# 9to1url/PairPhone

Measured on AMD Instinct MI355X. Metric: MELPe-1200 channel-seconds encoded/sec (node), higher is better.
Workload: dtype int16/int32 saturating fixed point; 1 GPU; config 4: 262144 channels per GPU, melpe_a per superframe (NPP x3 + MELPe-1200 analysis + 81-bit packing); channels_per_gpu=262144, channels_total=262144, parallelism=channel shards, 1 GPU(s), no collective

## Files before the change

pairphone_amd/build.py:

```python
import os
import subprocess
import sys

ROOT = os.path.dirname(os.path.dirname(os.path.abspath(__file__)))
CSRC = os.path.join(ROOT, "pairphone_amd", "csrc")
LIB = os.path.join(ROOT, "pairphone_amd", "libmelpe_amd.so")
EMU = os.path.join(ROOT, "build", "libmelpe_hostemu.so")
REF = "/root/reference/melpe"
HIPCC = os.environ.get("HIPCC", "/opt/rocm/bin/hipcc")
ARCH = os.environ.get("MELPE_ARCH", "gfx950")


def _run(cmd, **kw):
    print("+", " ".join(cmd), flush=True)
    subprocess.run(cmd, check=True, **kw)


def _newer(target, deps):
    if not os.path.exists(target):
        return True
    t = os.path.getmtime(target)
    return any(os.path.getmtime(d) > t for d in deps if os.path.exists(d))


def _sources():
    out = []
    for d in (CSRC, os.path.join(ROOT, "include")):
        for f in os.listdir(d):
            if f.endswith((".h", ".hip", ".cpp")):
                out.append(os.path.join(d, f))
    out.append(os.path.join(ROOT, "pairphone_amd", "data", "melpe_tables.bin"))
    return out


def build_oracle():
    if not os.path.isdir(REF):
        print("reference not present: using prebuilt oracle/_ref and committed tables")
        return
    _run(["make", "-s", "-C", os.path.join(ROOT, "oracle"), "-j8"])
    _run([sys.executable, os.path.join(ROOT, "oracle", "dump_tables.py")])


PROF_LIB = os.path.join(ROOT, "pairphone_amd", "libmelpe_amd_prof.so")


TUS = ("engine", "k_npp", "k_ana", "k_ana_mw", "k_harm", "k_dec", "k_r24", "k_dsp_eval", "k_par",
       "k_link")
HOT_TUS = ("k_npp", "k_ana", "k_ana_mw", "k_harm", "k_dec", "k_r24", "k_dsp_eval", "k_par", "k_link")
TU_FLAGS = {"k_ana": ["-mllvm", "-amdgpu-disable-unclustered-high-rp-reschedule"]}


def build_engine(force=False, prof=False, defs=(), out=None, tus_defs=None, hot=HOT_TUS, only=None):
    out = out or (PROF_LIB if prof else LIB)
    deps = _sources()
    if not force and not _newer(out, deps):
        return out
    blob = os.path.join(ROOT, "pairphone_amd", "data", "melpe_tables.bin")
    tag = os.path.splitext(os.path.basename(out))[0]
    objdir = os.path.join(ROOT, "build", "obj", tag)
    os.makedirs(objdir, exist_ok=True)
    common = [HIPCC, "-O3", "--offload-arch=" + ARCH, "-std=c++17", "-fPIC", "-c",
              "-Wno-unused-result", "-Wno-unused-value", '-DMELPE_TABLES_BIN="%s"' % blob] \
        + (["-DMELPE_PROF"] if prof else []) + ["-D" + d for d in defs] \
        + os.environ.get("MELPE_EXTRA_FLAGS", "").split()
    procs, objs = [], []
    for tu in TUS:
        o = os.path.join(objdir, tu + ".o")
        objs.append(o)
        if only is not None and tu not in only and os.path.exists(o):
            continue
        extra = (["-DMELPE_INLINE_ALL"] if tu in hot else []) + TU_FLAGS.get(tu, [])
        if tus_defs and tu in tus_defs:
            extra += ["-D" + d for d in tus_defs[tu]]
        cmd = common + extra + [os.path.join(CSRC, tu + ".hip"), "-o", o]
        print("+", " ".join(cmd), flush=True)
        procs.append((tu, subprocess.Popen(cmd)))
    bad = [tu for tu, p in procs if p.wait() != 0]
    if bad:
        raise RuntimeError("hipcc failed for " + ", ".join(bad))
    check_no_flat(objdir)
    tmp = out + ".tmp"
# ... 1 lines not shown
    os.replace(tmp, out)
    return out


LLVM_BIN = "/opt/rocm/lib/llvm/bin"


def device_disassembly(obj, arch=None):
    arch = arch or ARCH
    import tempfile
    with tempfile.TemporaryDirectory() as tmp:
        fat, elf = os.path.join(tmp, "fat.bin"), os.path.join(tmp, "dev.elf")
        subprocess.run(["objcopy", "--dump-section", ".hip_fatbin=" + fat, obj], check=True)
        for a in dict.fromkeys((arch, "gfx950")):
            r = subprocess.run([os.path.join(LLVM_BIN, "clang-offload-bundler"), "--unbundle", "--type=o",
                                "--input=" + fat, "--targets=hipv4-amdgcn-amd-amdhsa--" + a,
                                "--output=" + elf], capture_output=True)
            if r.returncode == 0 and os.path.getsize(elf) > 0:
                break
        else:
            raise RuntimeError("no gfx950 code object in " + obj)
        txt = subprocess.run([os.path.join(LLVM_BIN, "llvm-objdump"), "-d", "--no-show-raw-insn",
                              elf], check=True, capture_output=True, text=True).stdout
    out, cur = {}, None
    for line in txt.splitlines():
        if line.endswith(">:") and "<" in line:
            cur = line[line.index("<") + 1:-2]
            out[cur] = []
        elif cur and line.startswith("\t"):
            out[cur].append(line.strip())
    return out


NO_FLAT = ("k_enc_ana", "k_enc_harm", "k_enc_tail", "k_decode", "k_vad", "k_enc_npp", "k_npp",
           "k_demodulate", "k_enc24",
           "k_dec24", "k_helpers_eval", "k_stream", "k_dsp_eval", "k_parse", "k_par_tap")


def check_no_flat(objdir):
    bad = []
    for f in sorted(os.listdir(objdir)):
        if not f.endswith(".o"):
            continue
        for sym, ins in device_disassembly(os.path.join(objdir, f)).items():
            if any(k in sym for k in NO_FLAT):
                n = sum(1 for i in ins if i.startswith("flat_"))
                if n:
                    bad.append("%s: %d flat_ instructions" % (sym, n))
    if bad:
        raise RuntimeError("generic FLAT accesses in codec kernels: " + "; ".join(bad))


def build_hostemu(force=False):
    deps = _sources()
    if not force and not _newer(EMU, deps):
        return EMU
    os.makedirs(os.path.dirname(EMU), exist_ok=True)
    tmp = EMU + ".tmp"
    _run(["g++", "-O2", "-std=c++17", "-shared", "-fPIC", "-I" + CSRC,
          os.path.join(CSRC, "hostemu.cpp"), "-o", tmp])
    os.replace(tmp, EMU)
    return EMU


def build_opcount(force=False):
    out = os.path.join(ROOT, "build", "libmelpe_opcount.so")
    if not force and not _newer(out, _sources()):
# ... 32 lines not shown
```

pairphone_amd/csrc/encoder.h:

```cpp
#ifndef MELPE_ENCODER_H
#define MELPE_ENCODER_H

#include "quant.h"

namespace mlp {



MD void ana_first(EncAna *E)
{
	if (!E->ana_started) {
		v_zero(E->lpfsp_delin, LPF_ORD);
		v_zero(E->lpfsp_delout, LPF_ORD);
		E->pitch_avg = DEFAULT_PITCH_Q7;
		v_set(E->fpitch, DEFAULT_PITCH_Q7, 2);
		E->ana_started = 1;
	}
}

MN Word16 global_pitch(const int16_t *speech, int16_t *sb, int16_t *delin, int16_t *delout)
{
	Word16 dontcare;
#if !defined(MELPE_OPCOUNT)
	{
// ... 417 lines not shown
	window(E->sigbuf, TB(win_cof), E->sigbuf, LPC_FRAME);
	find_harm_fft(E->sigbuf, hb, LPC_FRAME);
}

MN void ana_pack(EncAna *E)
{
	MelpParam *par = E->par;
	quant_fsmag(E, par);
	for (int i = 0; i < NF; i++)
		E->qpar.uv_flag[i] = par[i].uv_flag;
	low_rate_chn_write(E);
	v_copy(E->hpspeech, &E->hpspeech[NF * FRAME], IN_BEG);
}

MN void analysis_tail(EncAna *E)
{
	MelpParam *par = E->par;
	sc_ana(E, par);
#if !defined(MELPE_KO_LSFVQ)
	lsf_vq(E, par);
#endif
	pitch_vq(E, par);
	gain_vq(E, par);
	for (int i = 0; i < NF; i++)
		quant_u(&par[i].jitter, &E->qpar.jit_index[i], 0, MAX_JITTER_Q15, 2, SW_MAX_,
			true, 7);
	quant_bp(E, par);
	quant_jitter(E, par);
	for (int i = 0; i < NF; i++)
		ana_fsmag_frame(E, &par[i], i);
	ana_pack(E);
}

MN void analysis_a2(EncAna *E, int16_t *res)
{
	MelpParam *par = E->par;
	sc_ana(E, par);
#if !defined(MELPE_KO_LSFVQ)
	lsf_vq(E, par);
#endif
	ANA_CKPT(4);
	pitch_vq(E, par);
	gain_vq(E, par);
	for (int i = 0; i < NF; i++)
		quant_u(&par[i].jitter, &E->qpar.jit_index[i], 0, MAX_JITTER_Q15, 2, SW_MAX_,
			true, 7);
	quant_bp(E, par);
	quant_jitter(E, par);
	for (int i = 0; i < NF; i++) {
		if (par[i].uv_flag)
			continue;
		int16_t lpc[LPC_ORD + 1];
		lpc[0] = 4096;
		lpc_lsp2pred(par[i].lsf, &lpc[1], LPC_ORD);
		zerflt(&E->hpspeech[i * FRAME + FRAME_END - LPC_FRAME / 2], lpc, E->sigbuf, LPC_ORD,
		       LPC_FRAME);
		window(E->sigbuf, TB(win_cof), E->sigbuf, LPC_FRAME);
		v_copy(&res[i * LPC_FRAME], E->sigbuf, LPC_FRAME);
	}
	v_copy(E->hpspeech, &E->hpspeech[NF * FRAME], IN_BEG);
}

MN void analysis_a(EncAna *E, const int16_t *sp_in, int16_t *res)
{
#if defined(MELPE_KO_ANALYSIS)
	return;
#endif
	for (int i = 0; i < NF; i++) {
		analysis_frame(E, sp_in, i);
		ANA_CKPT(i + 1);
	}
	analysis_a2(E, res);
}

MD void ana_shift(EncAna *E)
{
	v_copy(E->hpspeech, &E->hpspeech[NF * FRAME], IN_BEG);
}

MN void analysis_b(EncAna *E)
{
	MelpParam *par = E->par;
	quant_fsmag(E, par);
	for (int i = 0; i < NF; i++)
		E->qpar.uv_flag[i] = par[i].uv_flag;
	low_rate_chn_write(E);
}

MN void analysis(EncAna *E, const int16_t *sp_in)
{
	PROF_SCOPE(15);
#if defined(MELPE_KO_ANALYSIS)
	return;
#endif
	for (int i = 0; i < NF; i++)
		analysis_frame(E, sp_in, i);
	analysis_tail(E);
}

MN void analysis_upto(EncAna *E, const int16_t *sp_in, int upto)
{
	MelpParam *par = E->par;
	int16_t lpc[LPC_ORD + 1];
	for (int i = 0; i < NF; i++) {
		dc_rmv(&sp_in[i * FRAME], &E->hpspeech[IN_BEG + i * FRAME], E->dcdelin,
// ... 53 lines not shown
```

pairphone_amd/csrc/engine.hip:

```cpp
#include <hip/hip_runtime.h>
#include <stdio.h>
#include <stdlib.h>
#include <string.h>
#include <stdint.h>
#include <initializer_list>
#include <string>
#include <mutex>
#include <vector>

#include "kern.h"
#define SYN_FN __host__ __device__ static inline
#include "synth.h"
#include "voice_crypt.h"
#include "vad.h"
#include "stream_fmt.h"
#include "ops_eval.h"
#include "helpers_eval.h"
#include "dsp_eval_modes.h"
#define MODEM_FN __host__ __device__ static inline
#include "modem.h"
#include "../../include/melpe.h"
#include "../../include/melpe_batch.h"

#if !defined(__HIP_DEVICE_COMPILE__)
// ... 486 lines not shown
	hipEvent_t done = nullptr;
	hipStream_t last = nullptr;
	bool used = false;
};

static hipError_t bin_alloc(BinBuf *b, int channels)
{
	size_t pb = sizeof(int) * (size_t) channels, cb = sizeof(unsigned) * (2 * NBIN + 4);
	const size_t kb = sizeof(uint16_t) * (size_t) channels;
	char *p = nullptr;
	hipError_t er = hipMalloc(&p, pb + cb + kb);
	if (er != hipSuccess)
		return er;
	er = hipEventCreateWithFlags(&b->done, hipEventDisableTiming);
	if (er != hipSuccess) {
		hipFree(p);
		return er;
	}
	b->perm = (int *) p;
	b->ctl = (unsigned *) (p + pb);
	b->key = (uint16_t *) (p + pb + cb);
	return hipMemset(b->ctl, 0, cb);
}

__device__ __forceinline__ int bin_class(const char *rec, int off_par, int off_uv)
{
	const int16_t *uv = (const int16_t *) (rec + off_uv);
	const int nv = (uv[0] == 0) + (uv[1] == 0) + (uv[2] == 0);
	int b = (*(const int16_t *) (rec + off_par + (NF - 1) * sizeof(MelpParam)) >> 7) - 20;
	b = b < 0 ? 0 : (b > BIN_PITCHES - 1 ? BIN_PITCHES - 1 : b);
	return nv * BIN_PITCHES + b;
}

__global__ __launch_bounds__(256) void k_bin_count(const char *rec, size_t stride, int off_par,
						   int off_uv, const uint8_t *active, int n, BinBuf b)
{
	__shared__ unsigned cnt[NBIN];
	for (int k = threadIdx.x; k < NBIN; k += blockDim.x)
		cnt[k] = 0;
	__syncthreads();
	int c = blockIdx.x * blockDim.x + threadIdx.x;
	if (c < n) {
		int k = NOT_LIVE;
		if (!active || active[c]) {
			k = bin_class(rec + (size_t) c * stride, off_par, off_uv);
			atomicAdd(&cnt[k], 1u);
		}
		b.key[c] = (uint16_t) k;
	}
	__syncthreads();
	for (int k = threadIdx.x; k < NBIN; k += blockDim.x)
		if (cnt[k])
			atomicAdd(&b.ctl[k], cnt[k]);
}

__global__ void k_bin_scan(BinBuf b)
{
	if (threadIdx.x == 0) {
		unsigned acc = 0;
		for (int k = 0; k < NBIN; k++) {
			b.ctl[NBIN + k] = acc;
			acc += b.ctl[k];
		}
		b.ctl[2 * NBIN] = acc;
		b.ctl[2 * NBIN + 1] = 0;
		b.ctl[2 * NBIN + 2] = 0;
	}
}

__global__ __launch_bounds__(256) void k_bin_scatter(int n, BinBuf b)
{
	__shared__ unsigned cnt[NBIN], base[NBIN];
	for (int k = threadIdx.x; k < NBIN; k += blockDim.x)
		cnt[k] = 0;
	__syncthreads();
	int c = blockIdx.x * blockDim.x + threadIdx.x;
	int k = c < n ? b.key[c] : NOT_LIVE;
	unsigned r = 0;
	if (k != NOT_LIVE)
		r = atomicAdd(&cnt[k], 1u);
	__syncthreads();
	for (int j = threadIdx.x; j < NBIN; j += blockDim.x)
		if (cnt[j])
			base[j] = atomicAdd(&b.ctl[NBIN + j], cnt[j]);
	__syncthreads();
	if (k != NOT_LIVE)
		b.perm[base[k] + r] = c;
}

static bool bin_enabled(void)
{
	static const bool on = env_int("MELPE_BIN", 1) != 0;
	return on;
}

static hipError_t bin_launch(int order, BinBuf &b, const void *rec, size_t stride, int off_par,
			     int off_uv, const uint8_t *active, int n, hipStream_t s, bool *on)
{
	*on = !(order == 0 || (order < 0 && !bin_enabled()));
	if (!*on)
		return hipSuccess;
	hipError_t er;
	if (b.used && b.last != s && (er = hipStreamWaitEvent(s, b.done, 0)) != hipSuccess)
		return er;
	unsigned g = (unsigned) ((n + 255) / 256);
	if ((er = hipMemsetAsync(b.ctl, 0, sizeof(unsigned) * NBIN, s)) != hipSuccess)
		return er;
	k_bin_count<<<g, 256, 0, s>>>((const char *) rec, stride, off_par, off_uv, active, n, b);
	if ((er = hipGetLastError()) != hipSuccess)
		return er;
	k_bin_scan<<<1, WAVE, 0, s>>>(b);
	if ((er = hipGetLastError()) != hipSuccess)
		return er;
	k_bin_scatter<<<g, 256, 0, s>>>(n, b);
	return hipGetLastError();
}

static hipError_t bin_release(BinBuf &b, hipStream_t s)
{
	b.last = s;
	b.used = true;
	return hipEventRecord(b.done, s);
}

#define MW_MAX_CHANNELS (512 * WAVE)
#define DEC2_MAX_CHANNELS (1024 * WAVE)

struct melpe_engine {
	int device = 0;
	int channels = 0;
	hipStream_t stream = nullptr;
	hipEvent_t ev0 = nullptr, ev1 = nullptr;
	hipEvent_t ev_in = nullptr, ev_out = nullptr;
	hipEvent_t ev_host = nullptr;
	hipEvent_t ev_pin = nullptr, ev_npp = nullptr;
	EncState *d_enc = nullptr;
	DecState *d_dec = nullptr;
	synth_state *d_syn = nullptr;
	int16_t *d_pcm = nullptr;
	unsigned char *d_bits = nullptr;
	uint8_t *d_mask = nullptr;
	int16_t *d_npp = nullptr;
	BinBuf bin_enc, bin_dec;
	int lane_order = -1;
	int ana_waves = 0;
	uint32_t *d_lq = nullptr;
	int dec_waves = 0;
	uint32_t *d_hb = nullptr;
	int mw_live_max = MW_MAX_CHANNELS;
	size_t scratch_need = 0;
	int16_t *d_res = nullptr;
	std::vector<std::pair<hipStream_t, hipEvent_t>> marks;
	std::recursive_mutex mu;
	size_t npp_bytes = 0;
	float last_ms = 0.f;
	struct Slot {
		int16_t *pcm = nullptr;
		unsigned char *bits = nullptr;
		uint8_t *mask = nullptr;
		hipEvent_t loaded = nullptr, done = nullptr, freed = nullptr;
		bool used = false;
	} slot[2];
	hipStream_t cin = nullptr, cout = nullptr;
	hipStream_t cdec = nullptr;
	hipEvent_t ev_dec = nullptr;
	long async_calls = 0;
	hipStream_t own = nullptr;
};

static int ana_waves_for(melpe_engine *e)
{
	if (e->ana_waves == 1 || e->ana_waves == 4)
		return e->ana_waves;
	long groups = (e->channels + WAVE - 1) / WAVE;
	return groups <= 512 ? 4 : 1;
}

static int ana_launch(melpe_engine *e, const int16_t *d_sp, uint8_t *d_bits, const uint8_t *d_act,
		      hipStream_t s, hipEvent_t after_sort = nullptr)
{
	BinBuf &b = e->bin_enc;
	bool on;
	hipError_t er = bin_launch(e->lane_order, b, e->d_enc, sizeof(EncState),
				   (int) (offsetof(EncState, a) + offsetof(EncAna, par)),
				   (int) (offsetof(EncState, a) + offsetof(EncAna, qpar) + offsetof(QuantParam, uv_flag)),
				   d_act, e->channels, s, &on);
	if (er != hipSuccess)
		return (int) er;
	if (after_sort && (er = hipEventRecord(after_sort, s)) != hipSuccess)
		return (int) er;
	const int *perm = on ? b.perm : nullptr;
	const int *nlive = on ? (const int *) (b.ctl + 2 * NBIN) : nullptr;
	int nw = ana_waves_for(e);
	AnaGate all;
	all.tag = (int *) (b.ctl + 2 * NBIN + 1);
	const bool dual = nw == 1 && on && e->ana_waves == 0 && e->mw_live_max > 0;
	AnaGate lane = all, mw = all;
	if (dual) {
		lane.lo = e->mw_live_max;
		mw.hi = e->mw_live_max;
	}
	int rc = 0;
	if (dual || nw == 4)
		rc = kl_enc_ana_mw(e->d_enc, d_sp, d_bits, d_act, e->channels, perm, nlive, e->d_lq, mw, s);
	if (rc == 0 && nw == 1) {
		rc = kl_enc_ana(e->d_enc, d_sp, d_act, e->channels, perm, nlive, e->d_res, lane, s);
		if (rc == 0)
			rc = kl_enc_harm(e->d_enc, e->d_res, d_act, e->channels, perm, nlive, lane, s);
		if (rc == 0)
			rc = kl_enc_tail(e->d_enc, d_bits, d_act, e->channels, perm, nlive, lane, s);
	}
	if (rc == 0 && on)
		rc = (int) bin_release(b, s);
	return rc;
}

static int dec_waves_for(melpe_engine *e)
{
	int nw = e->dec_waves;
	if (nw != 1 && nw != 2)
		nw = e->channels <= DEC2_MAX_CHANNELS ? 2 : 1;
	return nw == 2 && e->d_hb ? 2 : 1;
}

static int dec_launch(melpe_engine *e, int16_t *d_sp, const uint8_t *d_bits, const uint8_t *d_act,
		      hipStream_t s)
{
	BinBuf &b = e->bin_dec;
	bool on;
	hipError_t er = bin_launch(e->lane_order, b, e->d_dec, sizeof(DecState),
				   (int) offsetof(DecState, par),
				   (int) (offsetof(DecState, qpar) + offsetof(QuantParam, uv_flag)),
				   d_act, e->channels, s, &on);
	if (er != hipSuccess)
		return (int) er;
	const int *perm = on ? b.perm : nullptr;
	const int *nlive = on ? (const int *) (b.ctl + 2 * NBIN) : nullptr;
	int rc = dec_waves_for(e) == 2
			 ? kl_decode2(e->d_dec, d_sp, d_bits, d_act, e->channels, perm, nlive, e->d_hb, s)
			 : kl_decode(e->d_dec, d_sp, d_bits, d_act, e->channels, perm, nlive, s);
	if (rc == 0 && on)
		rc = (int) bin_release(b, s);
	return rc;
// ... 270 lines not shown
			HIPCHK(hipStreamWaitEvent(e->cdec, e->ev_pin, 0));
			HIPCHK((hipError_t) dec_launch(e, (int16_t *) dc->sp, (const uint8_t *) dc->bits,
						       (const uint8_t *) dc->active, e->cdec));
			HIPCHK(hipEventRecord(e->ev_dec, e->cdec));
		}
		if (nx) {
			HIPCHK(hipStreamWaitEvent(e->cin, e->ev_pin, 0));
			if (nx->vad)
				if (int r = vad_launch(nx->vad, nx->sp, nx->votes, (void *) nx->mask, nx->active,
						       e->channels, e->cin))
					return r;
			HIPCHK((hipError_t) kl_enc_npp(e->d_enc, (int16_t *) nx->sp, (const uint8_t *) nx->mask,
						       e->channels, e->cin));
			HIPCHK(hipEventRecord(e->ev_npp, e->cin));
			HIPCHK(hipStreamWaitEvent(s, e->ev_npp, 0));
		}
		if (dc)
			HIPCHK(hipStreamWaitEvent(s, e->ev_dec, 0));
		return 0;
	});
}

extern "C" {

const char *melpe_last_error(void)
{
	return g_err.c_str();
}

static int engine_warm(melpe_engine *e)
{
	hipError_t er;
	const int mw = e->channels < MW_MAX_CHANNELS ? e->channels : MW_MAX_CHANNELS;
	int (*warm[])(int, hipStream_t) = {kl_npp_warm, kl_ana_warm, kl_harm_warm, kl_ana_mw_warm, kl_dec_warm};
	for (auto f : warm)
		if ((er = (hipError_t) f(f == kl_ana_mw_warm ? mw : e->channels, e->stream)) != hipSuccess)
			return fail("melpe_engine: codec kernel scratch could not be reserved", er);
	if (e->d_hb && (er = (hipError_t) kl_dec2_warm(e->channels, e->stream)) != hipSuccess)
		return fail("melpe_engine: codec kernel scratch could not be reserved", er);

	if ((er = hipStreamSynchronize(e->stream)) != hipSuccess)
		return fail("melpe_engine: codec kernel scratch could not be reserved", er);
	return 0;
}

static int engine_reserve(melpe_engine *e)
{
	DEVGUARD(e->device);
	hipError_t er;
	if ((er = hipMalloc(&e->d_res, sizeof(int16_t) * NF * LPC_FRAME * (size_t) e->channels)) != hipSuccess) {
		e->d_res = nullptr;
		return fail("melpe_engine_create: analysis residual buffer", er);
	}
	if ((er = hipMalloc(&e->d_lq, sizeof(uint32_t) * kl_enc_ana_mw_lq_words(e->channels))) != hipSuccess) {
		e->d_lq = nullptr;
		return fail("melpe_engine_create: multi-wave score rows", er);
	}
	if (e->channels <= DEC2_MAX_CHANNELS &&
	    (er = hipMalloc(&e->d_hb, sizeof(uint32_t) * kl_decode2_hb_words(e->channels))) != hipSuccess) {
		e->d_hb = nullptr;
		return fail("melpe_engine_create: two-wave decoder hand-over buffers", er);
	}
	const int mw = e->channels < MW_MAX_CHANNELS ? e->channels : MW_MAX_CHANNELS;
	{
		const size_t lane = kl_ana_private() > kl_harm_private() ? kl_ana_private() : kl_harm_private();
		const size_t dec_lane = kl_dec_private() > kl_parse_private() ? kl_dec_private() : kl_parse_private();
		const size_t per_wave = (lane > dec_lane ? lane : dec_lane) * WAVE;
		const size_t mw_wave = kl_ana_mw_private() * WAVE;
		const size_t ww = kl_npp_private() > kl_harm_wave_private() ? kl_npp_private() : kl_harm_wave_private();
		const size_t waves = (size_t) (e->channels + WAVE - 1) / WAVE;
		const size_t mw_waves = 4 * (size_t) ((mw + WAVE - 1) / WAVE);
		size_t resident = (size_t) e->channels;
		hipDeviceProp_t prop;
		if (hipGetDeviceProperties(&prop, e->device) == hipSuccess) {
			const size_t r = (size_t) prop.multiProcessorCount * (size_t) (prop.maxThreadsPerMultiProcessor / WAVE);
			if (r > 0 && r < resident)
				resident = r;
		}
		size_t need = per_wave * waves;
		if (mw_wave * mw_waves > need)
			need = mw_wave * mw_waves;
		if (e->d_hb && kl_dec2_private() * WAVE * 2 * waves > need)
			need = kl_dec2_private() * WAVE * 2 * waves;
		if (ww * WAVE * resident > need)
			need = ww * WAVE * resident;
		size_t cur = 0, mx = 0;
		if (hipDeviceGetLimit(&cur, hipExtLimitScratchCurrent) == hipSuccess &&
		    hipDeviceGetLimit(&mx, hipExtLimitScratchMax) == hipSuccess && need > cur) {
			if (need > mx)
				return fail_msg("melpe_engine_create: the codec kernels' scratch exceeds the "
						"device's scratch limit (fewer channels per engine)");
			if ((er = hipDeviceSetLimit(hipExtLimitScratchCurrent, need)) != hipSuccess)
				return fail("melpe_engine_create: raising the scratch limit", er);
		}
		e->scratch_need = need;
	}
	return engine_warm(e);
}
// ... 2 lines not shown
{
	if (!out || channels <= 0)
		return fail_msg("melpe_engine_create: bad arguments");
	int ndev = 0;
	HIPCHK(hipGetDeviceCount(&ndev));
	if (device < 0 || device >= ndev)
		return fail_msg("melpe_engine_create: no such HIP device");
	int rc = ensure_device_tables(device);
	if (rc)
		return rc;
	DEVGUARD(device);
	melpe_engine *e = new melpe_engine();
	e->device = device;
	e->channels = channels;
	hipError_t er = hipSuccess;
	const char *what = nullptr;
#define CREATE_STEP(expr) if (er == hipSuccess && (er = (expr)) != hipSuccess) what = #expr
	e->stream = g_dev_stream[device];
	CREATE_STEP(hipEventCreate(&e->ev0));
	CREATE_STEP(hipEventCreate(&e->ev1));
	CREATE_STEP(hipEventCreateWithFlags(&e->ev_in, hipEventDisableTiming));
	CREATE_STEP(hipEventCreateWithFlags(&e->ev_out, hipEventDisableTiming));
	CREATE_STEP(hipEventCreateWithFlags(&e->ev_host, hipEventDisableTiming));
	CREATE_STEP(hipEventCreateWithFlags(&e->ev_pin, hipEventDisableTiming));
	CREATE_STEP(hipEventCreateWithFlags(&e->ev_npp, hipEventDisableTiming));
	CREATE_STEP(hipMalloc(&e->d_enc, sizeof(EncState) * (size_t) channels));
	CREATE_STEP(hipMalloc(&e->d_dec, sizeof(DecState) * (size_t) channels));
	CREATE_STEP(hipMalloc(&e->d_syn, sizeof(synth_state) * (size_t) channels));
	CREATE_STEP(hipMalloc(&e->d_pcm, sizeof(int16_t) * MELPE_SF_SAMPLES * (size_t) channels));
	CREATE_STEP(hipMalloc(&e->d_bits, (size_t) MELPE_SF_BYTES * channels));
	CREATE_STEP(hipMalloc(&e->d_mask, (size_t) channels));
	CREATE_STEP(bin_alloc(&e->bin_enc, channels));
	CREATE_STEP(bin_alloc(&e->bin_dec, channels));
#undef CREATE_STEP
	if (er != hipSuccess) {
		int r = fail(what, er);
		melpe_engine_destroy(e);
		return r;
	}
	int r = melpe_engine_reset(e, nullptr, 3);
	if (r == 0)
		r = engine_reserve(e);
	if (r) {
		std::string m = g_err;
		melpe_engine_destroy(e);
		g_err = m;
		return r;
	}
	*out = e;
	return 0;
}

int melpe_engine_set_own_stream(melpe_engine *e, int on)
{
	if (!e)
		return fail_msg("melpe_engine_set_own_stream: null engine");
	DEVGUARD(e->device);
	HOST_LOCK(e);
	ENGINE_WAIT(e);
	HIPCHK(hipStreamSynchronize(e->stream));
	if (on && !e->own) {
		HIPCHK(hipStreamCreateWithFlags(&e->own, hipStreamNonBlocking));
		e->stream = e->own;
		if (int rc = engine_warm(e)) {
			e->stream = g_dev_stream[e->device];
			hipStreamDestroy(e->own);
// ... 43 lines not shown
		return fail_msg("melpe_engine_set_dec_waves: waves must be 0 (auto), 1 or 2");
	if (waves == 2 && !e->d_hb)
		return fail_msg("melpe_engine_set_dec_waves: the two-wave decoder is available up to "
				"65,536 channels per engine");
	std::lock_guard<std::recursive_mutex> lk(e->mu);
	e->dec_waves = waves;
	return 0;
}

int melpe_engine_set_ana_waves(melpe_engine *e, int waves)
{
	if (!e || !(waves == 0 || waves == 1 || waves == 4))
		return fail_msg("melpe_engine_set_ana_waves: waves must be 0 (auto), 1 or 4");
	std::lock_guard<std::recursive_mutex> lk(e->mu);
	e->ana_waves = waves;
	return 0;
}

int melpe_engine_destroy(melpe_engine *e)
{
	if (!e)
		return 0;
	DevGuard dg(e->device);
	engine_wait(e);
	hipFree(e->d_npp);
	hipFree(e->d_enc);
	hipFree(e->d_dec);
	hipFree(e->d_syn);
	hipFree(e->d_pcm);
	hipFree(e->d_bits);
	hipFree(e->d_mask);
	hipFree(e->bin_enc.perm);
	hipFree(e->bin_dec.perm);
	hipFree(e->d_lq);
	hipFree(e->d_hb);
	hipFree(e->d_res);
	for (auto &m : e->marks)
		hipEventDestroy(m.second);
	if (e->bin_enc.done)
		hipEventDestroy(e->bin_enc.done);
	if (e->bin_dec.done)
		hipEventDestroy(e->bin_dec.done);
	if (e->ev0)
		hipEventDestroy(e->ev0);
	if (e->ev1)
		hipEventDestroy(e->ev1);
	if (e->ev_in)
		hipEventDestroy(e->ev_in);
	if (e->ev_out)
		hipEventDestroy(e->ev_out);
	if (e->ev_host)
		hipEventDestroy(e->ev_host);
	if (e->ev_pin)
		hipEventDestroy(e->ev_pin);
	if (e->ev_npp)
		hipEventDestroy(e->ev_npp);
	for (auto &sl : e->slot) {
		hipFree(sl.pcm);
		hipFree(sl.bits);
		hipFree(sl.mask);
		for (hipEvent_t ev : {sl.loaded, sl.done, sl.freed})
			if (ev)
				hipEventDestroy(ev);
	}
	if (e->own)
		hipStreamDestroy(e->own);
	if (e->cin)
		hipStreamDestroy(e->cin);
	if (e->cout)
		hipStreamDestroy(e->cout);
	if (e->cdec)
		hipStreamDestroy(e->cdec);
	if (e->ev_dec)
		hipEventDestroy(e->ev_dec);
	delete e;
// ... 1097 lines not shown
```

pairphone_amd/csrc/hostemu.cpp:

```cpp
#include <stdio.h>
#include <stdlib.h>
#include <string.h>
#include <vector>

#include "codec.h"
#if !defined(MELPE_OPCOUNT)
#include "ana_mw.h"
#endif
#include "helpers_eval.h"
#include "dsp_eval.h"
#include "codec2400.h"
#include "voice_crypt.h"
#include "link.h"
#include "vad.h"
#include "modem.h"

using namespace mlp;

struct emu_engine {
	int channels;
	std::vector<EncState> enc;
	std::vector<DecState> dec;
};

// ... 50 lines not shown
{
	for (int c = 0; c < e->channels; c++)
		for (int f = 0; f < frames; f++) {
			int16_t *x = sp + (size_t) c * stride + f * NPP_HOP;
			npp_frame(&e->enc[c].npp, &g_npp_scratch, x, x, rate1200 != 0);
		}
	return 0;
}

int emu_encode(emu_engine *e, unsigned char *bits, int16_t *sp)
{
	for (int c = 0; c < e->channels; c++) {
		encode_superframe(&e->enc[c], &g_npp_scratch, sp + (size_t) c * BLOCK);
		for (int k = 0; k < 11; k++)
			bits[c * 11 + k] = e->enc[c].a.chbuf[k];
	}
	return 0;
}

int emu_encode_npp(emu_engine *e, int16_t *sp)
{
	for (int c = 0; c < e->channels; c++) {
		int16_t *x = sp + (size_t) c * BLOCK;
		for (int f = 0; f < NF; f++)
			npp_frame(&e->enc[c].npp, &g_npp_scratch, x + f * FRAME, x + f * FRAME);
	}
	return 0;
}

int emu_encode_ana_split(emu_engine *e, unsigned char *bits, const int16_t *sp)
{
	static int16_t res[NF * LPC_FRAME];
	static EncAna L;
	for (int c = 0; c < e->channels; c++) {
		EncAna *E = &L;
		for (int k = 0; k < NF * LPC_FRAME; k++)
			res[k] = (int16_t) 0x5a5a;
		memcpy(E, &e->enc[c].a, ENC_ANA_LIVE);
		memset((char *) E + ENC_ANA_LIVE, 0x5a + (c & 7), sizeof(EncAna) - ENC_ANA_LIVE);
		analysis_a(E, sp + (size_t) c * BLOCK, res);
		memcpy(&e->enc[c].a, E, ENC_ANA_LIVE);
		E = &e->enc[c].a;
		for (int i = 0; i < NF; i++) {
			MelpParam *par = &E->par[i];
			v_set(par->fs_mag, 8192, NUM_HARM);
			if (!par->uv_flag)
				find_harm(&res[i * LPC_FRAME], par->fs_mag, par->pitch, NUM_HARM, LPC_FRAME);
		}
		analysis_b(E);
		for (int k = 0; k < 11; k++)
			bits[c * 11 + k] = E->chbuf[k];
	}
	return 0;
}

int emu_encode_ana(emu_engine *e, unsigned char *bits, const int16_t *sp)
{
	for (int c = 0; c < e->channels; c++) {
		analysis(&e->enc[c].a, sp + (size_t) c * BLOCK);
		for (int k = 0; k < 11; k++)
			bits[c * 11 + k] = e->enc[c].a.chbuf[k];
	}
	return 0;
}

#if !defined(MELPE_OPCOUNT)
struct HostXch {
	int16_t w[XS_WORDS];
	int16_t get(int k) const { return w[k]; }
	void put(int k, int16_t v) { w[k] = v; }
};

struct HostDb {
	uint32_t v[LQ_ROW];
	uint32_t get(int u) const { return v[u]; }
// ... 421 lines not shown
```

pairphone_amd/csrc/k_ana.hip:

```cpp
#define MELPE_PROG_PRIO
#include "kern.h"

MELPE_TU(ana)

struct AnaLane {
	uint8_t guard[FLAT_GUARD_BYTES];
	EncAna S;
	int16_t x[BLOCK];
};

#if defined(MELPE_WAVE_TIMES)
__device__ unsigned long long g_wave_t[2 * 16384];
__device__ unsigned g_wave_hw[2 * 16384];
extern "C" int kl_wave_times(unsigned long long *out, int n)
{
	return (int) hipMemcpyFromSymbol(out, HIP_SYMBOL(g_wave_t), sizeof(unsigned long long) * n);
}
extern "C" int kl_wave_hw(unsigned *out, int n)
{
	return (int) hipMemcpyFromSymbol(out, HIP_SYMBOL(g_wave_hw), sizeof(unsigned) * n);
}
#define WT_START() const unsigned long long wt0_ = __builtin_amdgcn_s_memrealtime()
#define WT_END()                                                                         \
	do {                                                                             \
// ... 6 lines not shown
	} while (0)
#else
#define WT_START() (void) 0
#define WT_END() (void) 0
#endif

template <int MODE>
__global__ __launch_bounds__(WAVE, MELPE_ENC_WAVES) void k_enc_ana(EncState *enc, const int16_t *sp, uint8_t *bits,
						  const uint8_t *active, int n, const int *perm,
						  const int *nlive, int16_t *res, AnaGate gate, int prio)
{
	static_assert(MODE == 1, "the unsplit analysis (MODE 0) is gone");
	WT_START();
	int c = blockIdx.x * WAVE + threadIdx.x;
	if (perm) {
		const int L = *nlive;
		if (!gate.open(L))
			return;
		gate.mark(c == 0 && L > 0, 1);
		if (c >= L)
			return;
		PP_BEGIN(prio ? (unsigned *) (nlive + 2) : nullptr, (L + WAVE - 1) / WAVE);
		c = perm[c];
	} else {
		PP_BEGIN(nullptr, 1);
		gate.mark(c == 0, 1);
		if (c >= n || (active && !active[c]))
			return;
	}
	AnaLane L;
	PIN_FRAME(L);
	constexpr size_t nb = ENC_ANA_LIVE;
	static_assert(offsetof(AnaLane, S) % 16 == 0, "the record copy is in 16-byte pieces");
	lane_copy_x4(&L.S, &enc[c].a, nb);
	lane_copy(L.x, sp + (size_t) c * BLOCK, sizeof(int16_t) * BLOCK);
	analysis_a(&L.S, L.x, res + (size_t) c * NF * LPC_FRAME);
	lane_copy_x4(&enc[c].a, &L.S, nb);
	WT_END();
}

__global__ __launch_bounds__(WAVE, MELPE_ENC_WAVES) void k_enc_ana_dbg(EncState *enc, const int16_t *sp, int n, int upto)
{
	int c = blockIdx.x * WAVE + threadIdx.x;
	PP_BEGIN(nullptr, 1);
	if (c >= n || upto <= 0)
		return;
	AnaLane L;
	PIN_FRAME(L);
	lane_copy(&L.S, &enc[c].a, ENC_ANA_LIVE);
	lane_copy(L.x, sp + (size_t) c * BLOCK, sizeof(int16_t) * BLOCK);
	analysis_upto(&L.S, L.x, upto);
	lane_copy(&enc[c].a, &L.S, ENC_ANA_LIVE);
}

static int ana_prio_mode(void)
{
	static const int v = env_int("MELPE_ANA_PRIO", 1) != 0;
	return v;
}

static int launch_ana(int lanes, EncState *enc, const int16_t *sp, const uint8_t *active, int n, const int *perm,
		      const int *nlive, int16_t *res, AnaGate gate, int prio, hipStream_t s)
{
	k_enc_ana<1><<<grid_for(lanes), WAVE, 0, s>>>(enc, sp, nullptr, active, n, perm, nlive, res, gate, prio);
	return (int) hipGetLastError();
}

extern "C" int kl_enc_ana(EncState *enc, const int16_t *sp, const uint8_t *active, int n, const int *perm,
			  const int *nlive, int16_t *res, AnaGate gate, hipStream_t s)
// ... 21 lines not shown
```

pairphone_amd/csrc/launch.h:

```cpp
#ifndef MELPE_LAUNCH_H
#define MELPE_LAUNCH_H

#include <hip/hip_runtime.h>
#include <stddef.h>
#include <stdint.h>

namespace mlp {
struct EncState;
struct DecState;
}
struct AnaGate;
struct LinkState;

#define MELPE_TU_LIST(X) X(eng) X(npp) X(ana) X(anamw) X(harm) X(dec) X(r24) X(dspeval) X(par)

extern "C" {

#define MELPE_TU_DECL(name)                                      \
	int melpe_tu_##name##_upload(const void *blob, size_t bytes); \
	int melpe_tu_##name##_prof(uint64_t *acc);
MELPE_TU_LIST(MELPE_TU_DECL)
#undef MELPE_TU_DECL

int kl_npp(mlp::EncState *enc, int16_t *sp, int frames, int stride, const uint8_t *active, int n,
	   int rate1200, hipStream_t s);
int kl_enc_npp(mlp::EncState *enc, int16_t *sp, const uint8_t *active, int n, hipStream_t s);
int kl_dsp_scalar_lds(int mode, const int32_t *args, int32_t *out, long n, hipStream_t s);
int kl_dsp_wave_fft(int mode, const int16_t *in, const int32_t *args, int32_t *out, int n, hipStream_t s);

int kl_enc_ana(mlp::EncState *enc, const int16_t *sp, const uint8_t *active, int n, const int *perm,
	       const int *nlive, int16_t *res, AnaGate gate, hipStream_t s);
int kl_enc_ana_dbg(mlp::EncState *enc, const int16_t *sp, int n, int upto, hipStream_t s);

int kl_enc_harm(mlp::EncState *enc, const int16_t *res, const uint8_t *active, int n, const int *perm,
		const int *nlive, AnaGate gate, hipStream_t s);
int kl_enc_tail(mlp::EncState *enc, uint8_t *bits, const uint8_t *active, int n, const int *perm,
		const int *nlive, AnaGate gate, hipStream_t s);
int kl_dsp_wave_harm(const int16_t *in, const int32_t *args, int32_t *out, int n, hipStream_t s);

int kl_enc_ana_mw(mlp::EncState *enc, const int16_t *sp, uint8_t *bits, const uint8_t *active, int n,
		  const int *perm, const int *nlive, uint32_t *lqbuf, AnaGate gate, hipStream_t s);
size_t kl_enc_ana_mw_lq_words(int n);

int kl_decode(mlp::DecState *dec, int16_t *sp, const uint8_t *bits, const uint8_t *active, int n,
	      const int *perm, const int *nlive, hipStream_t s);
int kl_decode2(mlp::DecState *dec, int16_t *sp, const uint8_t *bits, const uint8_t *active, int n,
	       const int *perm, const int *nlive, uint32_t *hbuf, hipStream_t s);
size_t kl_decode2_hb_words(int n);

int kl_enc24(mlp::EncState *enc, const int16_t *sp, uint8_t *bits, const uint8_t *active, int n,
	     hipStream_t s);
int kl_dec24(mlp::DecState *dec, int16_t *sp, const uint8_t *bits, const uint8_t *active, int n,
	     hipStream_t s);

int kl_dsp_eval(int mode, const int16_t *in, const int32_t *args, int32_t *out, int n, hipStream_t s);
int kl_dsp_scalar(int mode, const int32_t *args, int32_t *out, long n, hipStream_t s);

int kl_par_tap(const char *rec, size_t stride, size_t off, uint32_t *par, uint32_t *qpar,
	       const uint8_t *active, int n, hipStream_t s);
int kl_parse(mlp::DecState *dec, uint32_t *par, const uint8_t *bits, const uint8_t *active, int n,
	     hipStream_t s);

int kl_link_tx(LinkState *st, uint8_t *pkts, const uint8_t *voiced, int32_t *ret, const uint8_t *active,
	       int channels, int packets, hipStream_t s);
int kl_link_rx(LinkState *st, uint8_t *pkts, int32_t *ret, uint8_t *voice, const uint8_t *active,
	       int channels, int packets, hipStream_t s);
int kl_golay_sweep(uint32_t *enc, uint64_t *digest, hipStream_t s);

size_t kl_npp_private(void);
size_t kl_ana_private(void);
size_t kl_harm_private(void);
size_t kl_harm_wave_private(void);
size_t kl_ana_mw_private(void);
size_t kl_dec_private(void);
size_t kl_dec2_private(void);
size_t kl_parse_private(void);
int kl_npp_warm(int n, hipStream_t s);
int kl_ana_warm(int n, hipStream_t s);
int kl_harm_warm(int n, hipStream_t s);
int kl_ana_mw_warm(int n, hipStream_t s);
int kl_dec_warm(int n, hipStream_t s);
int kl_dec2_warm(int n, hipStream_t s);

}

#endif
```

Baseline: 522,300 channel-s/s.

## Split encoder analysis into a separate quantisation kernel with voicing-class lane re-sort

Moves the quantisation stage (LSF/pitch/gain VQ and residual windowing) out of the per-lane analysis kernel into a new k_enc_quant kernel. Analysis now writes a span of hpspeech into the residual buffer, and the quantiser rebuilds that span from it. Between the two kernels, lanes are re-binned by the three frames' voicing flags so that wavefronts running the quantiser and later stages share control flow. It also forces the single-wave dual path when the multi-wave count would otherwise be four. This adds kernel launches, a second sort, and extra global traffic for copying record slices and the span, in exchange for less divergence and possibly higher occupancy.

Measured after the change: 534,100 channel-s/s, median of 6. +2.3%, better.

```diff
diff --git a/pairphone_amd/build.py b/pairphone_amd/build.py
--- a/pairphone_amd/build.py
+++ b/pairphone_amd/build.py
@@ -44,9 +44,9 @@
 PROF_LIB = os.path.join(ROOT, "pairphone_amd", "libmelpe_amd_prof.so")
 
 
-TUS = ("engine", "k_npp", "k_ana", "k_ana_mw", "k_harm", "k_dec", "k_r24", "k_dsp_eval", "k_par",
+TUS = ("engine", "k_npp", "k_ana", "k_quant", "k_ana_mw", "k_harm", "k_dec", "k_r24", "k_dsp_eval", "k_par",
        "k_link")
-HOT_TUS = ("k_npp", "k_ana", "k_ana_mw", "k_harm", "k_dec", "k_r24", "k_dsp_eval", "k_par", "k_link")
+HOT_TUS = ("k_npp", "k_ana", "k_quant", "k_ana_mw", "k_harm", "k_dec", "k_r24", "k_dsp_eval", "k_par", "k_link")
 TU_FLAGS = {"k_ana": ["-mllvm", "-amdgpu-disable-unclustered-high-rp-reschedule"]}
 
 
@@ -114,7 +114,7 @@
     return out
 
 
-NO_FLAT = ("k_enc_ana", "k_enc_harm", "k_enc_tail", "k_decode", "k_vad", "k_enc_npp", "k_npp",
+NO_FLAT = ("k_enc_ana", "k_enc_quant", "k_enc_harm", "k_enc_tail", "k_decode", "k_vad", "k_enc_npp", "k_npp",
            "k_demodulate", "k_enc24",
            "k_dec24", "k_helpers_eval", "k_stream", "k_dsp_eval", "k_parse", "k_par_tap")
 
diff --git a/pairphone_amd/csrc/encoder.h b/pairphone_amd/csrc/encoder.h
--- a/pairphone_amd/csrc/encoder.h
+++ b/pairphone_amd/csrc/encoder.h
@@ -473,14 +473,36 @@
 	ana_pack(E);
 }
 
-MN void analysis_a2(EncAna *E, int16_t *res)
-{
+#define ANA_RES_BEG (FRAME_END - LPC_FRAME / 2 - LPC_ORD)
+#define ANA_RES_END ((NF - 1) * FRAME + FRAME_END + LPC_FRAME / 2)
+#define ANA_XSPAN_BEG (ANA_RES_BEG & ~7)
+#define ANA_XSPAN_END ((ANA_RES_END + 7) & ~7)
+#define ANA_XSPAN_BYTES (sizeof(int16_t) * (ANA_XSPAN_END - ANA_XSPAN_BEG))
+static_assert(ANA_XSPAN_END <= IN_BEG + BLOCK && ANA_XSPAN_END - ANA_XSPAN_BEG <= NF * LPC_FRAME,
+	      "the residual span lies in hpspeech and fits a row of the residual buffer");
+static_assert((sizeof(int16_t) * NF * LPC_FRAME) % 16 == 0, "rows of the residual buffer in 16-byte pieces");
+
+MN void analysis_a1(EncAna *E, const int16_t *sp_in)
+{
+#if defined(MELPE_KO_ANALYSIS)
+	return;
+#endif
+	for (int i = 0; i < NF; i++) {
+		analysis_frame(E, sp_in, i);
+		ANA_CKPT(i + 1);
+	}
+	sc_ana(E, E->par);
+}
+
+MN void analysis_q(EncAna *E, int16_t *res)
+{
+#if defined(MELPE_KO_ANALYSIS)
+	return;
+#endif
 	MelpParam *par = E->par;
-	sc_ana(E, par);
 #if !defined(MELPE_KO_LSFVQ)
 	lsf_vq(E, par);
 #endif
-	ANA_CKPT(4);
 	pitch_vq(E, par);
 	gain_vq(E, par);
 	for (int i = 0; i < NF; i++)
@@ -499,19 +521,6 @@
 		window(E->sigbuf, TB(win_cof), E->sigbuf, LPC_FRAME);
 		v_copy(&res[i * LPC_FRAME], E->sigbuf, LPC_FRAME);
 	}
-	v_copy(E->hpspeech, &E->hpspeech[NF * FRAME], IN_BEG);
-}
-
-MN void analysis_a(EncAna *E, const int16_t *sp_in, int16_t *res)
-{
-#if defined(MELPE_KO_ANALYSIS)
-	return;
-#endif
-	for (int i = 0; i < NF; i++) {
-		analysis_frame(E, sp_in, i);
-		ANA_CKPT(i + 1);
-	}
-	analysis_a2(E, res);
 }
 
 MD void ana_shift(EncAna *E)
diff --git a/pairphone_amd/csrc/engine.hip b/pairphone_amd/csrc/engine.hip
--- a/pairphone_amd/csrc/engine.hip
+++ b/pairphone_amd/csrc/engine.hip
@@ -542,6 +542,15 @@
 	return nv * BIN_PITCHES + b;
 }
 
+#define KEY_PITCH 0
+#define KEY_VOICING 1
+__device__ __forceinline__ int bin_class_uvc(const char *rec, int off_par)
+{
+	const MelpParam *par = (const MelpParam *) (rec + off_par);
+	return (par[0].uv_flag ? 4 : 0) | (par[1].uv_flag ? 2 : 0) | (par[2].uv_flag ? 1 : 0);
+}
+
+template <int KEY>
 __global__ __launch_bounds__(256) void k_bin_count(const char *rec, size_t stride, int off_par,
 						   int off_uv, const uint8_t *active, int n, BinBuf b)
 {
@@ -553,7 +562,8 @@
 	if (c < n) {
 		int k = NOT_LIVE;
 		if (!active || active[c]) {
-			k = bin_class(rec + (size_t) c * stride, off_par, off_uv);
+			k = KEY == KEY_VOICING ? bin_class_uvc(rec + (size_t) c * stride, off_par)
+					       : bin_class(rec + (size_t) c * stride, off_par, off_uv);
 			atomicAdd(&cnt[k], 1u);
 		}
 		b.key[c] = (uint16_t) k;
@@ -604,19 +614,29 @@
 	return on;
 }
 
+static hipError_t bin_prepare(BinBuf &b, hipStream_t s)
+{
+	hipError_t er;
+	if (b.used && b.last != s && (er = hipStreamWaitEvent(s, b.done, 0)) != hipSuccess)
+		return er;
+	return hipMemsetAsync(b.ctl, 0, sizeof(unsigned) * NBIN, s);
+}
+
 static hipError_t bin_launch(int order, BinBuf &b, const void *rec, size_t stride, int off_par,
-			     int off_uv, const uint8_t *active, int n, hipStream_t s, bool *on)
+			     int off_uv, const uint8_t *active, int n, hipStream_t s, bool *on,
+			     int key = KEY_PITCH, bool prepared = false)
 {
 	*on = !(order == 0 || (order < 0 && !bin_enabled()));
 	if (!*on)
 		return hipSuccess;
 	hipError_t er;
-	if (b.used && b.last != s && (er = hipStreamWaitEvent(s, b.done, 0)) != hipSuccess)
+	if (!prepared && (er = bin_prepare(b, s)) != hipSuccess)
 		return er;
 	unsigned g = (unsigned) ((n + 255) / 256);
-	if ((er = hipMemsetAsync(b.ctl, 0, sizeof(unsigned) * NBIN, s)) != hipSuccess)
-		return er;
-	k_bin_count<<<g, 256, 0, s>>>((const char *) rec, stride, off_par, off_uv, active, n, b);
+	if (key == KEY_VOICING)
+		k_bin_count<KEY_VOICING><<<g, 256, 0, s>>>((const char *) rec, stride, off_par, off_uv, active, n, b);
+	else
+		k_bin_count<KEY_PITCH><<<g, 256, 0, s>>>((const char *) rec, stride, off_par, off_uv, active, n, b);
 	if ((er = hipGetLastError()) != hipSuccess)
 		return er;
 	k_bin_scan<<<1, WAVE, 0, s>>>(b);
@@ -652,6 +672,7 @@
 	uint8_t *d_mask = nullptr;
 	int16_t *d_npp = nullptr;
 	BinBuf bin_enc, bin_dec;
+	BinBuf bin_enc2;
 	int lane_order = -1;
 	int ana_waves = 0;
 	uint32_t *d_lq = nullptr;
@@ -697,14 +718,21 @@
 				   d_act, e->channels, s, &on);
 	if (er != hipSuccess)
 		return (int) er;
-	if (after_sort && (er = hipEventRecord(after_sort, s)) != hipSuccess)
-		return (int) er;
 	const int *perm = on ? b.perm : nullptr;
 	const int *nlive = on ? (const int *) (b.ctl + 2 * NBIN) : nullptr;
 	int nw = ana_waves_for(e);
 	AnaGate all;
 	all.tag = (int *) (b.ctl + 2 * NBIN + 1);
-	const bool dual = nw == 1 && on && e->ana_waves == 0 && e->mw_live_max > 0;
+	bool dual = nw == 1 && on && e->ana_waves == 0 && e->mw_live_max > 0;
+	if (nw == 4 && on && e->ana_waves == 0 && e->mw_live_max > 0 && e->mw_live_max < e->channels) {
+		dual = true;
+		nw = 1;
+	}
+	BinBuf &b2 = e->bin_enc2;
+	if (on && nw == 1 && (er = bin_prepare(b2, s)) != hipSuccess)
+		return (int) er;
+	if (after_sort && (er = hipEventRecord(after_sort, s)) != hipSuccess)
+		return (int) er;
 	AnaGate lane = all, mw = all;
 	if (dual) {
 		lane.lo = e->mw_live_max;
@@ -715,10 +743,22 @@
 		rc = kl_enc_ana_mw(e->d_enc, d_sp, d_bits, d_act, e->channels, perm, nlive, e->d_lq, mw, s);
 	if (rc == 0 && nw == 1) {
 		rc = kl_enc_ana(e->d_enc, d_sp, d_act, e->channels, perm, nlive, e->d_res, lane, s);
+		if (rc == 0 && on) {
+			bool on2;
+			rc = (int) bin_launch(1, b2, e->d_enc, sizeof(EncState),
+					      (int) (offsetof(EncState, a) + offsetof(EncAna, par)), 0, d_act,
+					      e->channels, s, &on2, KEY_VOICING, true);
+			perm = b2.perm;
+			nlive = (const int *) (b2.ctl + 2 * NBIN);
+		}
+		if (rc == 0)
+			rc = kl_enc_quant(e->d_enc, e->d_res, d_act, e->channels, perm, nlive, lane, s);
 		if (rc == 0)
 			rc = kl_enc_harm(e->d_enc, e->d_res, d_act, e->channels, perm, nlive, lane, s);
 		if (rc == 0)
 			rc = kl_enc_tail(e->d_enc, d_bits, d_act, e->channels, perm, nlive, lane, s);
+		if (rc == 0 && on)
+			rc = (int) bin_release(b2, s);
 	}
 	if (rc == 0 && on)
 		rc = (int) bin_release(b, s);
@@ -1055,7 +1095,8 @@
 {
 	hipError_t er;
 	const int mw = e->channels < MW_MAX_CHANNELS ? e->channels : MW_MAX_CHANNELS;
-	int (*warm[])(int, hipStream_t) = {kl_npp_warm, kl_ana_warm, kl_harm_warm, kl_ana_mw_warm, kl_dec_warm};
+	int (*warm[])(int, hipStream_t) = {kl_npp_warm, kl_ana_warm, kl_quant_warm, kl_harm_warm, kl_ana_mw_warm,
+						    kl_dec_warm};
 	for (auto f : warm)
 		if ((er = (hipError_t) f(f == kl_ana_mw_warm ? mw : e->channels, e->stream)) != hipSuccess)
 			return fail("melpe_engine: codec kernel scratch could not be reserved", er);
@@ -1086,7 +1127,9 @@
 	}
 	const int mw = e->channels < MW_MAX_CHANNELS ? e->channels : MW_MAX_CHANNELS;
 	{
-		const size_t lane = kl_ana_private() > kl_harm_private() ? kl_ana_private() : kl_harm_private();
+		size_t lane = kl_ana_private() > kl_harm_private() ? kl_ana_private() : kl_harm_private();
+		if (kl_quant_private() > lane)
+			lane = kl_quant_private();
 		const size_t dec_lane = kl_dec_private() > kl_parse_private() ? kl_dec_private() : kl_parse_private();
 		const size_t per_wave = (lane > dec_lane ? lane : dec_lane) * WAVE;
 		const size_t mw_wave = kl_ana_mw_private() * WAVE;
@@ -1155,6 +1198,7 @@
 	CREATE_STEP(hipMalloc(&e->d_mask, (size_t) channels));
 	CREATE_STEP(bin_alloc(&e->bin_enc, channels));
 	CREATE_STEP(bin_alloc(&e->bin_dec, channels));
+	CREATE_STEP(bin_alloc(&e->bin_enc2, channels));
 #undef CREATE_STEP
 	if (er != hipSuccess) {
 		int r = fail(what, er);
@@ -1264,6 +1308,7 @@
 	hipFree(e->d_mask);
 	hipFree(e->bin_enc.perm);
 	hipFree(e->bin_dec.perm);
+	hipFree(e->bin_enc2.perm);
 	hipFree(e->d_lq);
 	hipFree(e->d_hb);
 	hipFree(e->d_res);
@@ -1273,6 +1318,8 @@
 		hipEventDestroy(e->bin_enc.done);
 	if (e->bin_dec.done)
 		hipEventDestroy(e->bin_dec.done);
+	if (e->bin_enc2.done)
+		hipEventDestroy(e->bin_enc2.done);
 	if (e->ev0)
 		hipEventDestroy(e->ev0);
 	if (e->ev1)
diff --git a/pairphone_amd/csrc/hostemu.cpp b/pairphone_amd/csrc/hostemu.cpp
--- a/pairphone_amd/csrc/hostemu.cpp
+++ b/pairphone_amd/csrc/hostemu.cpp
@@ -106,15 +106,30 @@
 {
 	static int16_t res[NF * LPC_FRAME];
 	static EncAna L;
-	for (int c = 0; c < e->channels; c++) {
-		EncAna *E = &L;
+	static EncAna Q;
+	const size_t o = offsetof(EncAna, par), n = offsetof(EncAna, voicedEn) - o;
+	const size_t o2 = offsetof(EncAna, pvq_prev_uv_flag), n2 = offsetof(EncAna, fsm_prev_uv) - o2;
+	for (int c = 0; c < e->channels; c++) {
+		EncAna *E = &L, *R = &e->enc[c].a;
+		memcpy(E, R, ENC_ANA_LIVE);
+		memset((char *) E + ENC_ANA_LIVE, 0x5a + (c & 7), sizeof(EncAna) - ENC_ANA_LIVE);
+		analysis_a1(E, sp + (size_t) c * BLOCK);
 		for (int k = 0; k < NF * LPC_FRAME; k++)
 			res[k] = (int16_t) 0x5a5a;
-		memcpy(E, &e->enc[c].a, ENC_ANA_LIVE);
-		memset((char *) E + ENC_ANA_LIVE, 0x5a + (c & 7), sizeof(EncAna) - ENC_ANA_LIVE);
-		analysis_a(E, sp + (size_t) c * BLOCK, res);
-		memcpy(&e->enc[c].a, E, ENC_ANA_LIVE);
-		E = &e->enc[c].a;
+		memcpy(res, &E->hpspeech[ANA_RES_BEG], sizeof(int16_t) * (ANA_RES_END - ANA_RES_BEG));
+		ana_shift(E);
+		memcpy(R, E, ENC_ANA_LIVE);
+		E = &Q;
+		memset(E, 0xa5 - (c & 7), sizeof(EncAna));
+		memcpy((char *) E + o, (const char *) R + o, n);
+		memcpy((char *) E + o2, (const char *) R + o2, n2);
+		memcpy(&E->hpspeech[ANA_RES_BEG], res, sizeof(int16_t) * (ANA_RES_END - ANA_RES_BEG));
+		for (int k = 0; k < NF * LPC_FRAME; k++)
+			res[k] = (int16_t) 0x5a5a;
+		analysis_q(E, res);
+		memcpy((char *) R + o, (const char *) E + o, n);
+		memcpy((char *) R + o2, (const char *) E + o2, n2);
+		E = R;
 		for (int i = 0; i < NF; i++) {
 			MelpParam *par = &E->par[i];
 			v_set(par->fs_mag, 8192, NUM_HARM);
diff --git a/pairphone_amd/csrc/k_ana.hip b/pairphone_amd/csrc/k_ana.hip
--- a/pairphone_amd/csrc/k_ana.hip
+++ b/pairphone_amd/csrc/k_ana.hip
@@ -62,9 +62,13 @@
 	PIN_FRAME(L);
 	constexpr size_t nb = ENC_ANA_LIVE;
 	static_assert(offsetof(AnaLane, S) % 16 == 0, "the record copy is in 16-byte pieces");
+	static_assert((offsetof(AnaLane, S) + offsetof(EncAna, hpspeech) + sizeof(int16_t) * ANA_XSPAN_BEG) % 16 == 0,
+		      "and so is the span copy");
 	lane_copy_x4(&L.S, &enc[c].a, nb);
 	lane_copy(L.x, sp + (size_t) c * BLOCK, sizeof(int16_t) * BLOCK);
-	analysis_a(&L.S, L.x, res + (size_t) c * NF * LPC_FRAME);
+	analysis_a1(&L.S, L.x);
+	lane_copy_x4(res + (size_t) c * NF * LPC_FRAME, &L.S.hpspeech[ANA_XSPAN_BEG], ANA_XSPAN_BYTES);
+	ana_shift(&L.S);
 	lane_copy_x4(&enc[c].a, &L.S, nb);
 	WT_END();
 }
diff --git a/pairphone_amd/csrc/k_quant.hip b/pairphone_amd/csrc/k_quant.hip
--- /dev/null
+++ b/pairphone_amd/csrc/k_quant.hip
@@ -0,0 +1,68 @@
+#include "kern.h"
+
+MELPE_TU(quant)
+
+#ifndef MELPE_QUANT_WAVES
+#define MELPE_QUANT_WAVES 4
+#endif
+
+struct QuantLane {
+	uint8_t guard[FLAT_GUARD_BYTES];
+	EncAna S;
+};
+
+__global__ __launch_bounds__(WAVE, MELPE_QUANT_WAVES) void k_enc_quant(EncState *enc, int16_t *res,
+									const uint8_t *active, int n,
+									const int *perm, const int *nlive,
+									AnaGate gate)
+{
+	int c = blockIdx.x * WAVE + threadIdx.x;
+	if (perm) {
+		const int L = *nlive;
+		if (!gate.open(L) || c >= L)
+			return;
+		c = perm[c];
+	} else if (c >= n || (active && !active[c])) {
+		return;
+	}
+	QuantLane L;
+	PIN_FRAME(L);
+	constexpr size_t o = offsetof(EncAna, par), e = offsetof(EncAna, voicedEn);
+	constexpr size_t o2 = offsetof(EncAna, pvq_prev_uv_flag) & ~(size_t) 3;
+	constexpr size_t e2 = (offsetof(EncAna, fsm_prev_uv) + 3) & ~(size_t) 3;
+	static_assert(o % 4 == 0 && e % 4 == 0, "the quantisers' record ranges are dword copies");
+	static_assert((offsetof(QuantLane, S) + offsetof(EncAna, hpspeech) + sizeof(int16_t) * ANA_XSPAN_BEG) % 16 == 0 &&
+			      ANA_XSPAN_BYTES % 16 == 0,
+		      "the span copy is in 16-byte pieces");
+	EncAna *R = &enc[c].a;
+	int16_t *row = res + (size_t) c * NF * LPC_FRAME;
+	lane_copy((char *) &L.S + o, (const char *) R + o, e - o);
+	lane_copy((char *) &L.S + o2, (const char *) R + o2, e2 - o2);
+	lane_copy_x4(&L.S.hpspeech[ANA_XSPAN_BEG], row, ANA_XSPAN_BYTES);
+	analysis_q(&L.S, row);
+	lane_copy((char *) R + o, (const char *) &L.S + o, e - o);
+	lane_copy((char *) R + o2, (const char *) &L.S + o2, e2 - o2);
+}
+
+static int launch_quant(int lanes, EncState *enc, int16_t *res, const uint8_t *active, int n,
+			const int *perm, const int *nlive, AnaGate gate, hipStream_t s)
+{
+	k_enc_quant<<<grid_for(lanes), WAVE, 0, s>>>(enc, res, active, n, perm, nlive, gate);
+	return (int) hipGetLastError();
+}
+
+extern "C" int kl_enc_quant(EncState *enc, int16_t *res, const uint8_t *active, int n, const int *perm,
+			    const int *nlive, AnaGate gate, hipStream_t s)
+{
+	return launch_quant(n, enc, res, active, n, perm, nlive, gate, s);
+}
+
+extern "C" size_t kl_quant_private(void)
+{
+	return private_bytes((const void *) k_enc_quant);
+}
+
+extern "C" int kl_quant_warm(int n, hipStream_t s)
+{
+	return launch_quant(n, nullptr, nullptr, nullptr, 0, nullptr, nullptr, AnaGate{}, s);
+}
diff --git a/pairphone_amd/csrc/launch.h b/pairphone_amd/csrc/launch.h
--- a/pairphone_amd/csrc/launch.h
+++ b/pairphone_amd/csrc/launch.h
@@ -12,7 +12,7 @@
 struct AnaGate;
 struct LinkState;
 
-#define MELPE_TU_LIST(X) X(eng) X(npp) X(ana) X(anamw) X(harm) X(dec) X(r24) X(dspeval) X(par)
+#define MELPE_TU_LIST(X) X(eng) X(npp) X(ana) X(quant) X(anamw) X(harm) X(dec) X(r24) X(dspeval) X(par)
 
 extern "C" {
 
@@ -31,6 +31,9 @@
 int kl_enc_ana(mlp::EncState *enc, const int16_t *sp, const uint8_t *active, int n, const int *perm,
 	       const int *nlive, int16_t *res, AnaGate gate, hipStream_t s);
 int kl_enc_ana_dbg(mlp::EncState *enc, const int16_t *sp, int n, int upto, hipStream_t s);
+
+int kl_enc_quant(mlp::EncState *enc, int16_t *res, const uint8_t *active, int n, const int *perm,
+		 const int *nlive, AnaGate gate, hipStream_t s);
 
 int kl_enc_harm(mlp::EncState *enc, const int16_t *res, const uint8_t *active, int n, const int *perm,
 		const int *nlive, AnaGate gate, hipStream_t s);
@@ -69,6 +72,7 @@
 
 size_t kl_npp_private(void);
 size_t kl_ana_private(void);
+size_t kl_quant_private(void);
 size_t kl_harm_private(void);
 size_t kl_harm_wave_private(void);
 size_t kl_ana_mw_private(void);
@@ -77,6 +81,7 @@
 size_t kl_parse_private(void);
 int kl_npp_warm(int n, hipStream_t s);
 int kl_ana_warm(int n, hipStream_t s);
+int kl_quant_warm(int n, hipStream_t s);
 int kl_harm_warm(int n, hipStream_t s);
 int kl_ana_mw_warm(int n, hipStream_t s);
 int kl_dec_warm(int n, hipStream_t s);
```
